# rahul003/dmlc-core

Hardware: AMD Instinct MI355X
Metric: parsed rows/sec (LibSVM->CSR in device memory), aggregate over GPUs (higher is better)
Workload: dtype fp32 values / u32 indices (text parse, no matmul)

## Files before the change

### src/gpu/tile_kernels.hip

```cpp
#include <dmlc/gpu/hip_utils.h>
#include <hip/hip_runtime.h>

#include <cstdlib>
#include <type_traits>

#include "../data/strtonum.h"
#include "./device_common.h"
#include "./kernels.h"
#include "./token_decode.h"

namespace dmlc {
namespace gpu {

namespace {
constexpr int kThreads = 256;
constexpr int kSub = static_cast<int>(kTileBytes / 4096);
constexpr unsigned kOffBits = 13;
constexpr unsigned kMaxTileTokens = static_cast<unsigned>(kTileBytes / 2);
static_assert(kTileBytes == 8192, "entry packing assumes 8 KiB tiles");

__device__ __forceinline__ uint32_t gather_hi(uint32_t z) {
  return __builtin_amdgcn_udot4(z, 0x08040201u, 0u, false) >> 7;
}

// ... 23 lines not shown
  for (int i = 0; i < 4; ++i) m |= gather_hi((w[i] << 1) & 0x80808080u) << (4 * i);
  return m;
}

__device__ __forceinline__ bool num_start(uint32_t c) {
  return (c >= '0' && c <= '9') || c == '+' || c == '-' || c == '.';
}

template <bool kCheck, bool kFull = false, bool kCheckTokens = true>
__device__ __forceinline__ bool lane_masks(uint4 v, uint32_t pc, size_t pos, size_t n,
                                           uint32_t* lm, uint32_t* tm) {
  uint32_t sep, eol, ctl;
  classify16(v, &sep, &eol, &ctl);
  const uint32_t prev_eol = (pc == '\n' || pc == '\r') ? 1u : 0u;
  const uint32_t prev_sep = (prev_eol || pc == ' ' || pc == '\t') ? 1u : 0u;
  uint32_t valid = 0xFFFFu;
  if (kFull) {
  } else if (pos >= n) {
    valid = 0;
  } else if (n - pos < 16) {
    valid = (1u << (n - pos)) - 1u;
  }
  *lm = ~eol & ((eol << 1) | prev_eol) & valid & 0xFFFFu;
  *tm = ~sep & ((sep << 1) | prev_sep) & valid & 0xFFFFu;
  if (!kCheck) return false;
  bool bad = (*lm & ~*tm) != 0;
  uint32_t t = kCheckTokens ? *tm : 0u;
  while (t != 0) {
    const int j = __ffs(t) - 1;
    t &= t - 1;
    bad |= !num_start(dev::vec_byte(v, j));
  }
  uint32_t c = ctl & valid;
  while (c != 0) {
    const int j = __ffs(c) - 1;
    c &= c - 1;
    bad |= !((0x2600u >> dev::vec_byte(v, j)) & 1u);
  }
  return bad;
}

__device__ __forceinline__ uint4 load16(const uint8_t* __restrict__ text, size_t pos, size_t n) {
  if (pos < n) return *reinterpret_cast<const uint4*>(text + pos);
  return make_uint4(0, 0, 0, 0);
}

__device__ __forceinline__ uint32_t prev_byte(const uint8_t* __restrict__ text, size_t pos,
                                              uint4 v) {
  const uint32_t from_left = dev::lane_shr1(v.w >> 24);
  if (dev::lane_id() != 0) return from_left;
  return pos == 0 ? static_cast<uint32_t>('\n') : text[pos - 1];
}

template <bool kFull>
__device__ __forceinline__ bool count16(uint4 v, uint32_t pc, size_t pos, size_t n,
                                        uint32_t* lines, uint32_t* toks, uint32_t* qtoks,
                                        uint32_t* packed = nullptr) {
  const uint32_t w[4] = {v.x, v.y, v.z, v.w};
  uint32_t acc_t[2] = {0u, 0u}, acc_l[2] = {0u, 0u};
  const size_t room = kFull ? 16 : (pos >= n ? 0 : (n - pos < 16 ? n - pos : 16));
  uint32_t prev_sep = (pc <= 0x20u) ? 0x80u : 0u;
  uint32_t prev_eol = (pc == '\n' || pc == '\r') ? 0x80u : 0u;
  bool bad = false;
  uint32_t blank = 0;
#pragma unroll
  for (int i = 0; i < 4; ++i) {
    const uint32_t x = w[i];
    const uint32_t lo7 = x & 0x7F7F7F7Fu;
    const uint32_t le20 = ~((lo7 + 0x5F5F5F5Fu) | x) & 0x80808080u;
    const uint32_t lt20 = ~((lo7 + 0x60606060u) | x) & 0x80808080u;
    const uint32_t b6 = ((x & 0x06060606u) + 0x7E7E7E7Eu) & 0x80808080u;
    const int valid_bytes = static_cast<int>(room) - 4 * i;
    const uint32_t valid = valid_bytes >= 4 ? 0x80808080u
                           : (valid_bytes <= 0 ? 0u : (0x80808080u >> (8 * (4 - valid_bytes))));
    const uint32_t sep = le20 | (~valid & 0x80808080u);
    const uint32_t eol = le20 & b6;
    const uint32_t sep_before = (sep << 8) | prev_sep;
    const uint32_t eol_before = (eol << 8) | prev_eol;
    const uint32_t tm = ~sep & sep_before & 0x80808080u;
    const uint32_t lm = ~eol & eol_before & valid & 0x80808080u;
    *qtoks += __popc(tm & (x << 1));
    const uint32_t wgt = (i & 1) ? 0x80402010u : 0x08040201u;
    acc_t[i >> 1] = __builtin_amdgcn_udot4(tm, wgt, acc_t[i >> 1], false);
    acc_l[i >> 1] = __builtin_amdgcn_udot4(lm, wgt, acc_l[i >> 1], false);
    blank |= lm & ~tm;
    uint32_t c = lt20 & valid;
    while (c != 0) {
      const int j = (__ffs(c) - 1) >> 3;
      c &= c - 1;
      bad |= !((0x2600u >> ((x >> (8 * j)) & 0xFFu)) & 1u);
    }
    prev_sep = (sep >> 24) & 0x80u;
    prev_eol = (eol >> 24) & 0x80u;
  }
  const uint32_t pt = (acc_t[0] >> 7) | (acc_t[1] << 1);
  const uint32_t pl = (acc_l[0] >> 7) | (acc_l[1] << 1);
  *toks += __popc(pt);
  *lines += __popc(pl);
  bad |= blank != 0;
  if (packed != nullptr) *packed = pt | (pl << 16);
  return bad;
}

template <bool kFull>
__device__ __forceinline__ uint32_t lines16(uint4 v, uint32_t pc, int room) {
  const uint32_t w[4] = {v.x, v.y, v.z, v.w};
  uint32_t prev_eol = (pc == '\n' || pc == '\r') ? 0x80u : 0u;
  uint32_t lines = 0;
#pragma unroll
  for (int i = 0; i < 4; ++i) {
    const uint32_t x = w[i];
    const uint32_t lo7 = x & 0x7F7F7F7Fu;
    const uint32_t le20 = ~((lo7 + 0x5F5F5F5Fu) | x) & 0x80808080u;
    const uint32_t b6 = ((x & 0x06060606u) + 0x7E7E7E7Eu) & 0x80808080u;
    const uint32_t eol = le20 & b6;
    const int valid_bytes = room - 4 * i;
    const uint32_t valid = kFull || valid_bytes >= 4
                               ? 0x80808080u
                               : (valid_bytes <= 0 ? 0u : (0x80808080u >> (8 * (4 - valid_bytes))));
    lines += __popc(~eol & ((eol << 8) | prev_eol) & valid);
    prev_eol = (eol >> 24) & 0x80u;
  }
  return lines;
}

__device__ __forceinline__ uint64_t lookback_lines(uint64_t* st, size_t tile, uint32_t own,
                                                   uint32_t tag, int lane) {
  const uint64_t tg = static_cast<uint64_t>(tag) << 34;
  if (lane == 0) {
    __hip_atomic_store(&st[tile], tg | ((tile == 0 ? 2ull : 1ull) << 32) | own, __ATOMIC_RELAXED,
                       __HIP_MEMORY_SCOPE_AGENT);
  }
  if (tile == 0) return 0;
  uint64_t excl = 0;
  int64_t j = static_cast<int64_t>(tile) - 1;
  for (;;) {
    const int64_t k = j - lane;
    const uint64_t v = k >= 0 ? __hip_atomic_load(&st[k], __ATOMIC_RELAXED, __HIP_MEMORY_SCOPE_AGENT)
                              : (tg | (2ull << 32));
    const uint32_t state = static_cast<uint32_t>(v >> 32) & 3u;
    const bool ready = (v >> 34) == tag && state != 0;
    const uint64_t inc = __ballot(ready && state == 2u);
    const uint64_t waiting = __ballot(!ready);
    const int first = inc != 0 ? __builtin_ctzll(inc) : dev::kWave - 1;
    const uint64_t need = first >= dev::kWave - 1 ? ~0ull : ((2ull << first) - 1ull);
    if ((waiting & need) != 0) {
      __builtin_amdgcn_s_sleep(1);
      continue;
    }
    excl += dev::wave_sum(lane <= first ? static_cast<uint32_t>(v) : 0u);
    if (inc != 0) break;
    j -= dev::kWave;
  }
  if (lane == 0) {
    __hip_atomic_store(&st[tile], tg | (2ull << 32) | (excl + own), __ATOMIC_RELAXED,
                       __HIP_MEMORY_SCOPE_AGENT);
  }
  return excl;
}

constexpr int kCountLoads = static_cast<int>(kTileBytes / 1024);
__global__ __launch_bounds__(kThreads) void k_tile_count(const uint8_t* __restrict__ text,
                                                         size_t n, size_t ntiles,
                                                         uint64_t* __restrict__ counts,
                                                         uint32_t* __restrict__ flags,
                                                         uint2* __restrict__ masks) {
  const int lane = dev::lane_id();
  const size_t tile = static_cast<size_t>(blockIdx.x) * (kThreads / dev::kWave) +
                      threadIdx.x / dev::kWave;
  if (tile >= ntiles) return;
  const size_t base = tile * kTileBytes;
  uint4 v[kCountLoads];
#pragma unroll
  for (int j = 0; j < kCountLoads; ++j) v[j] = load16(text, base + j * 1024 + lane * 16, n);
  const uint32_t first = base == 0 ? static_cast<uint32_t>('\n') : text[base - 1];
  uint32_t lines = 0, toks = 0, qtoks = 0;
  bool bad = false;
  uint2* const mrow = masks + tile * (kTileBytes / 2048) * dev::kWave + lane;
  auto count_tile = [&](auto full) {
    uint32_t m0 = 0;
#pragma unroll
    for (int j = 0; j < kCountLoads; ++j) {
      const uint32_t left = dev::lane_shr1(v[j].w >> 24);
      const uint32_t wrap = j == 0 ? first : dev::lane63(v[j - 1].w >> 24);
      const uint32_t pc = lane == 0 ? wrap : left;
      uint32_t m;
      bad |= count16<decltype(full)::value>(v[j], pc, base + j * 1024 + lane * 16, n, &lines,
                                            &toks, &qtoks, &m);
      if (j & 1) {
        mrow[(j >> 1) * dev::kWave] = make_uint2(m0, m);
      } else {
        m0 = m;
      }
    }
  };
  if (base + kTileBytes <= n) {
    count_tile(std::true_type{});
  } else {
    count_tile(std::false_type{});
  }
  lines = dev::wave_sum(lines);
  toks = dev::wave_sum(toks);
  qtoks = dev::wave_sum(qtoks);
  const bool any_bad = __any(bad);
  if (lane == 0) {
    counts[tile] = (static_cast<uint64_t>(lines) << 32) | (toks - qtoks);
    flags[tile] = (any_bad ? kFlagIrregular : 0u) | (qtoks != 0 ? kFlagQid : 0u);
  }
}

__device__ __forceinline__ void publish_host_meta(ChunkMeta* host_meta, ChunkMeta m) {
  m.pad = 0;
  *host_meta = m;
  __threadfence_system();
  *reinterpret_cast<volatile unsigned*>(&host_meta->pad) = 1u;
}

constexpr int kScanThreads = 1024;
constexpr int kScanPer = 8;

__global__ __launch_bounds__(kScanThreads) void k_tile_scan(uint64_t* __restrict__ counts,
                                                            const uint32_t* __restrict__ flags,
                                                            size_t ntiles, ChunkMeta* meta,
                                                            ChunkMeta* host_meta, int raw) {
  __shared__ uint64_t swave[kScanThreads / 64];
  __shared__ uint32_t sflag[kScanThreads / 64];
  const int wid = threadIdx.x / dev::kWave;
  uint64_t carry = 0;
  uint32_t fl = 0;
  for (size_t t0 = 0; t0 < ntiles; t0 += static_cast<size_t>(kScanThreads) * kScanPer) {
    const size_t base = t0 + static_cast<size_t>(threadIdx.x) * kScanPer;
    uint64_t v[kScanPer];
    uint64_t s = 0;
#pragma unroll
    for (int i = 0; i < kScanPer; ++i) {
      v[i] = base + i < ntiles ? counts[base + i] : 0;
      if (base + i < ntiles) fl |= flags[base + i];
      s += v[i];
    }
    uint64_t wtot;
    const uint64_t wx = dev::wave_excl_scan(s, &wtot);
    if (dev::lane_id() == 0) swave[wid] = wtot;
    __syncthreads();
    uint64_t before = 0, all = 0;
#pragma unroll
    for (int w = 0; w < kScanThreads / 64; ++w) {
      const uint64_t t = swave[w];
      if (w < wid) before += t;
      all += t;
    }
    uint64_t x = carry + before + wx;
#pragma unroll
    for (int i = 0; i < kScanPer; ++i) {
      if (base + i < ntiles) counts[base + i] = x;
      x += v[i];
    }
// ... 340 lines not shown
__device__ __forceinline__ void list_slice(uint32_t* sl, uint32_t tm, uint32_t lm, uint32_t at,
                                           uint32_t base, uint32_t line0, int lane) {
  uint32_t m = tm;
#pragma unroll
  for (int t = 0; t < 2; ++t) {
    const uint32_t j = static_cast<uint32_t>(__builtin_ctz(m | 0x10000u));
    const bool has = m != 0;
    sl[has ? at : kCap + lane] = list_entry(j & 15u, lm, base, line0);
    at += has ? 1u : 0u;
    m &= m - 1;
  }
  if (__any(m != 0)) {
    for (; m != 0; m &= m - 1) {
      sl[at++] = list_entry(static_cast<uint32_t>(__builtin_ctz(m)), lm, base, line0);
    }
  }
}

__device__ __forceinline__ uint32_t round_slot(int lane) {
  const uint32_t l = static_cast<uint32_t>(lane) & 31u;
  uint32_t k;
  if (l < 4) {
    k = l;
  } else if (l < 12) {
    k = 16u + (l - 4u);
  } else if (l < 16) {
    k = 4u + (l - 12u);
  } else if (l < 20) {
    k = 24u + (l - 16u);
  } else if (l < 28) {
    k = 8u + (l - 20u);
  } else {
    k = 28u + (l - 28u);
  }
  return (static_cast<uint32_t>(lane) & 32u) + k;
}

struct FillPass {
  uint64_t* status;
  unsigned long long* ticket;
  unsigned long long ticket0;
  ChunkMeta* meta;
  uint32_t exp;
  const uint32_t* masks;
};

template <TextFormat F, typename IndexType, bool kOnePass, bool kLean = false>
__global__ __launch_bounds__(kThreads, DMLC_FILL_WAVES) void k_tile_fill(
    const uint8_t* __restrict__ text, size_t n, size_t ntiles, const uint64_t* __restrict__ prefix,
    FillTarget<IndexType> out, MetaPartial* __restrict__ partials, FillPass op) {
  __shared__ uint4 s_text[kFillWaves][kStageVecs];
  __shared__ uint32_t s_list[kFillWaves][kListCap + 64];
  __shared__ uint32_t s_dq[kFillWaves][kQueueCap];
  const int wave = __builtin_amdgcn_readfirstlane(threadIdx.x / dev::kWave);
  const int lane = dev::lane_id();
  size_t group = blockIdx.x;
  if constexpr (kOnePass) {
    __shared__ uint32_t s_ticket;
    if (threadIdx.x == 0) s_ticket = static_cast<uint32_t>(atomicAdd(op.ticket, 1ull) - op.ticket0);
    __syncthreads();
    group = s_ticket;
  }
  const size_t tile = group * kFillWaves + wave;
  if (tile >= ntiles) return;
  uint4* const st = s_text[wave];
  uint32_t* const sl = s_list[wave];
  uint32_t* const dq = s_dq[wave];
  uint32_t qh = 0, qn = 0;
  const uint32_t slot = round_slot(lane);
  const size_t tile0 = tile * kTileBytes;

  const __amdgpu_buffer_rsrc_t trs = text_rsrc(text + tile0, n - tile0);
  const uint32_t loff = static_cast<uint32_t>(lane) * 16;
  uint4 a = bload16(trs, loff);
  uint4 b = bload16(trs, loff + 1024);
  uint4 t = make_uint4(0, 0, 0, 0);
  if (!kOnePass && lane < 4) t = bload16(trs, loff + kStepBytes);
  __amdgpu_buffer_rsrc_t mrs;
  const uint32_t moff = static_cast<uint32_t>(lane) * 8;
  uint2 mk = make_uint2(0, 0);
  if constexpr (!kOnePass) {
    mrs = mask_rsrc(op.masks, tile, ntiles);
    mk = load_masks(mrs, moff, 0);
  }
  uint32_t carry_pc = 0;
  if constexpr (kOnePass) carry_pc = tile0 == 0 ? static_cast<uint32_t>('\n') : text[tile0 - 1];
  uint64_t line_base, tok_base;
  unsigned count_flags = 0;
  if constexpr (kOnePass) {
    uint4 v[kCountLoads];
    v[0] = a;
    v[1] = b;
#pragma unroll
    for (int j = 2; j < kCountLoads; ++j) v[j] = bload16(trs, loff + j * 1024);
    if (lane < 4) t = v[2];
    uint32_t lines = 0, toks = 0, qtoks = 0;
    bool bad = false;
    auto count_tile = [&](auto full) {
#pragma unroll
      for (int j = 0; j < kCountLoads; ++j) {
        const uint32_t left = dev::lane_shr1(v[j].w >> 24);
        const uint32_t wrap = j == 0 ? carry_pc : dev::lane63(v[j - 1].w >> 24);
        const uint32_t pc = lane == 0 ? wrap : left;
        bad |= count16<decltype(full)::value>(v[j], pc, tile0 + j * 1024 + lane * 16, n, &lines,
                                              &toks, &qtoks);
      }
    };
    if (tile0 + kTileBytes <= n) {
      count_tile(std::true_type{});
    } else {
      count_tile(std::false_type{});
    }
    lines = dev::wave_sum(lines);
    const uint32_t ent = dev::wave_sum(toks - qtoks);
    qtoks = dev::wave_sum(qtoks);
    count_flags = (__any(bad) ? kFlagIrregular : 0u) | (qtoks != 0 ? kFlagQid : 0u);
    const uint64_t own = (static_cast<uint64_t>(lines) << 31) | ent;
    const uint64_t excl = dev::lookback_pairs<31>(op.status, tile, own, lane);
    line_base = excl >> 31;
    tok_base = excl & 0x7FFFFFFFull;
    if (tile + 1 == ntiles && lane == 0) {
      ChunkMeta m;
      m.nlines = m.nrows = line_base + lines;
      m.nnz = tok_base + ent - (line_base + lines);
      m.max_index = m.max_field = 0;
      m.flags = 0;
      m.pad = 0;
      *op.meta = m;
    }
  } else {
    const uint64_t pre = prefix[tile];
    line_base = pre >> 32;
    tok_base = pre & 0xffffffffull;
  }
  const uint64_t C = out.nnz_base + tok_base - line_base;
  const uint64_t R = out.row_base + line_base;
  auto clamp32 = [](int64_t v) {
    return static_cast<int32_t>(v > INT32_MAX ? INT32_MAX : (v < INT32_MIN ? INT32_MIN : v));
  };
  const int32_t nnz_room =
      clamp32(static_cast<int64_t>(out.nnz_limit) - static_cast<int64_t>(C));
  const int32_t row_room =
      clamp32(static_cast<int64_t>(out.row_limit) - static_cast<int64_t>(R));
  const uint32_t nnz_room_u = nnz_room > 0 ? static_cast<uint32_t>(nnz_room) : 0u;
  IndexType* const idx_at = out.index + C;
  float* const val_at = out.value + C;
  IndexType* const fld_at = out.field != nullptr ? out.field + C : nullptr;
  float* const lab_at = out.label + R - 1;
  uint64_t* const off_at = out.offset + R - 1;
  float* const wgt_at = !kLean && out.weight != nullptr ? out.weight + R - 1 : nullptr;
  uint64_t* const qid_at = !kLean && out.qid != nullptr ? out.qid + R - 1 : nullptr;
  const bool qid_chunk = !kLean && F == TextFormat::kLibSVM && out.qid != nullptr;

  uint32_t tok0 = 0;
  uint32_t lcnt = 0;
  uint32_t carry = 0;
  uint32_t qid_prev = 0;
  using MaxT = typename std::conditional<sizeof(IndexType) == 4, uint32_t, uint64_t>::type;
  MaxT mx_index = 0, mx_field = 0;
  bool any_value = false, any_weight = false, irregular = false, neg = false, need_w = false;
  bool over = false;
  uint32_t sink = 0;

#pragma unroll 1
  for (int s = 0; s < kSteps; ++s) {
    const bool last = s + 1 == kSteps;
    const size_t pos_a = tile0 + s * kStepBytes + lane * 16;
    if (tile0 + static_cast<size_t>(s + 1) * kStepBytes + 64 > n) {
// ... 119 lines not shown
      const uint32_t voff = static_cast<uint32_t>(rel) * 4u;
      auto at = [](auto* base, uint32_t off) {
        using T = typename std::remove_pointer<decltype(base)>::type;
        return reinterpret_cast<T*>(reinterpret_cast<char*>(base) + off);
      };
      if constexpr (F == TextFormat::kLibSVM) {
        if (feat) {
          *at(idx_at, boff) = static_cast<IndexType>(u0);
          *at(val_at, voff) = t.r == 2 ? t.f0 : 1.0f;
        }
        any_value |= feat && t.r == 2;
        const MaxT iu = static_cast<MaxT>(static_cast<IndexType>(u0));
        mx_index = feat && iu > mx_index ? iu : mx_index;
      } else {
        const uint64_t u1 = (static_cast<uint64_t>(t.u1_hi) << 32) | t.u1;
        if (feat) {
          *at(fld_at, boff) = static_cast<IndexType>(u0);
          *at(idx_at, boff) = static_cast<IndexType>(u1);
          *at(val_at, voff) = t.r == 3 ? t.f0 : 1.0f;
        }
        any_value |= feat && t.r == 3;
        const MaxT iu = static_cast<MaxT>(static_cast<IndexType>(u1));
        const MaxT fu = static_cast<MaxT>(static_cast<IndexType>(u0));
        mx_index = feat && iu > mx_index ? iu : mx_index;
        mx_field = feat && fu > mx_field ? fu : mx_field;
      }
      neg |= active && bad;
    };
    auto enqueue = [&](bool defer, uint32_t li) {
      const uint64_t dm = __ballot(defer);
      if (dm != 0) {
        const uint32_t rank = static_cast<uint32_t>(__popcll(dm & ((1ull << lane) - 1ull)));
        if (defer) dq[(qh + qn + rank) & (kQueueCap - 1)] = li;
        qn += static_cast<uint32_t>(__popcll(dm));
      }
    };
    for (uint32_t r0 = 0;;) {
      const bool qround = qn >= static_cast<uint32_t>(dev::kWave) || (r0 >= ndec && qn != 0);
      if (!qround && r0 >= ndec) break;
      if (!qround && r0 + 2 * dev::kWave <= ndec) {
        const uint32_t la = r0 + slot, lb = la + dev::kWave;
        const uint32_t ea = sl[la], eb = sl[lb];
        tok::Token ta, tb;
        ta.u0_hi = ta.u1_hi = tb.u0_hi = tb.u1_hi = 0;
        ta.u1 = tb.u1 = 0;
        bool oka, okb;
        if (dev::pricing_exp(op.exp) & 2u) {
          ta.u0 = ea;
          tb.u0 = eb;
          ta.f0 = ta.f1 = tb.f0 = tb.f1 = 1.0f;
          ta.r = tb.r = 2;
          oka = okb = true;
        } else {
          tok::decode2<F>(st, ea & 0x1FFFu, eb & 0x1FFFu, ((ea >> 13) & 1u) != 0,
                          ((eb >> 13) & 1u) != 0, &ta, &tb, &oka, &okb);
        }
        enqueue(!oka, la);
        enqueue(!okb, lb);
        emit(oka, ea, tok0 + la, ta, false);
        emit(okb, eb, tok0 + lb, tb, false);
        r0 += 2 * dev::kWave;
        continue;
      }
      bool active;
      uint32_t e, i;
      tok::Token t;
      t.u0_hi = t.u1_hi = 0;
      t.u1 = 0;
      bool bad = false;
      if (!qround) {
        const uint32_t li = r0 + slot;
        active = li < ndec;
        e = active ? sl[li] : 0u;
        i = tok0 + li;
        const bool is_label = active && ((e >> 13) & 1u) != 0;
        const bool ok = tok::decode<F>(st, e & 0x1FFFu, is_label, &t);
        enqueue(active & !ok, li);
        active = active & ok;
        r0 += dev::kWave;
      } else {
        dev::wave_sync();
        const uint32_t cnt = qn < static_cast<uint32_t>(dev::kWave) ? qn : dev::kWave;
        active = slot < cnt;
        const uint32_t li = active ? dq[(qh + slot) & (kQueueCap - 1)] : 0u;
        qh += cnt;
        qn -= cnt;
        e = active ? sl[li] : 0u;
        i = tok0 + li;
        const bool is_label = active && ((e >> 13) & 1u) != 0;
        const uint32_t off = e & 0x1FFFu;
        bool ok = false;
        if (active) {
          const tok::ExtToken x = tok::decode_ext<F>(
              st, off, is_label, off >= kSlotBytes ? 2 * kSlotBytes : kSlotBytes);
          t = x.t;
          ok = x.ok;
        }
        if (active & !ok) {
          const uint32_t in_slot = off >= kSlotBytes ? 1u : 0u;
          const int step = in_slot == (static_cast<uint32_t>(s) & 1u) ? s : s - 1;
          const size_t gpos =
              tile0 + static_cast<size_t>(step) * kStepBytes + off - in_slot * kSlotBytes;
          const GenericResult g = generic_token<F, IndexType>(text, n, gpos, is_label);
          t = g.t;
          bad = g.bad;
          irregular |= !num_start(text[gpos]);
        }
      }
      emit(active, e, i, t, bad);
    }
    const uint32_t left = total - ndec;
    const uint32_t moved = lane < static_cast<int>(left) ? sl[ndec + lane] : 0u;
    dev::wave_sync();
    if (lane < static_cast<int>(left)) sl[lane] = moved;
    tok0 += ndec;
    carry = left;
    lcnt += nline;
    dev::wave_sync();
  }
  unsigned fl = count_flags;
  if (sink == 0x9E3779B9u) fl |= kFlagIrregular;
  if (any_value) fl |= kFlagValue;
  if (any_weight) fl |= kFlagWeight;
  if (irregular) fl |= kFlagIrregular;
  if (neg) fl |= kFlagNegIndex;
  if (kLean ? any_weight : need_w) fl |= kFlagNeedWeight;
  if (over) fl |= kFlagOverflow;
  if (F == TextFormat::kLibFM) fl |= kFlagField;
  const unsigned long long mi = dev::wave_max(static_cast<unsigned long long>(mx_index));
  const unsigned long long mf = dev::wave_max(static_cast<unsigned long long>(mx_field));
  fl = dev::wave_or(fl);
  if (lane == 0) {
    MetaPartial p;
    p.max_index = mi;
    p.max_field = mf;
    p.flags = fl;
    p.pad = 0;
    partials[tile] = p;
  }
}

struct HashTarget {
  void* x;
  float* label;
  uint64_t row_base;
  uint64_t nlines;
  int dim;
  float scale;
  uint32_t seed;
  uint32_t tag;
  uint64_t* status;
  unsigned long long* ticket;
  unsigned long long ticket0;
  uint64_t row_cap;
  ChunkMeta* meta;
  const uint32_t* masks;
};

__device__ __forceinline__ uint32_t owned_tokens(uint32_t tm, uint32_t lm, uint32_t L0,
                                                 uint32_t own) {
  uint32_t m = tm;
  if (L0 == 0) m &= lm != 0 ? ~((lm & (0u - lm)) - 1u) : 0u;
  const uint32_t nl = static_cast<uint32_t>(__popc(lm));
  if (L0 + nl > own) {
    if (L0 > own) return 0u;
    uint32_t x = lm;
    for (uint32_t k = own - L0; k != 0; --k) x &= x - 1u;
    m &= (x & (0u - x)) - 1u;
  }
  return m;
}

template <TextFormat F, typename IndexType, bool kFP8, bool kOnePass>
__global__ __launch_bounds__(kThreads, DMLC_FILL_WAVES) void k_tile_hash(
    const uint8_t* __restrict__ text, size_t n, size_t ntiles,
    const uint64_t* __restrict__ prefix, HashTarget out, MetaPartial* __restrict__ partials) {
  __shared__ uint4 s_text[kFillWaves][kHashText / 16];
  __shared__ uint32_t s_list[kFillWaves][kHashListCap + 64];
  extern __shared__ __attribute__((aligned(16))) float s_hrow[];
  const int wave = __builtin_amdgcn_readfirstlane(threadIdx.x / dev::kWave);
  const int lane = dev::lane_id();
  size_t group = blockIdx.x;
  if constexpr (kOnePass) {
    __shared__ uint32_t s_ticket;
    if (threadIdx.x == 0) s_ticket = static_cast<uint32_t>(atomicAdd(out.ticket, 1ull) - out.ticket0);
    __syncthreads();
    group = s_ticket;
  }
  const size_t tile = group * kFillWaves + wave;
  if (tile >= ntiles) return;
  uint4* const st = s_text[wave];
  uint32_t* const sl = s_list[wave];
  const int dim = out.dim;
  float* const row = s_hrow + static_cast<size_t>(wave) * dim;
  const uint32_t slot = round_slot(lane);
  const size_t tile0 = tile * kTileBytes;
  const __amdgpu_buffer_rsrc_t trs = text_rsrc(text + tile0, n - tile0);
  const uint32_t loff = static_cast<uint32_t>(lane) * 16;
  uint4 a = bload16(trs, loff);
  uint4 b = bload16(trs, loff + 1024);
  __amdgpu_buffer_rsrc_t mrs;
  const uint32_t moff = static_cast<uint32_t>(lane) * 8;
  uint2 mk = make_uint2(0, 0);
  if constexpr (!kOnePass) {
    mrs = mask_rsrc(out.masks, tile, ntiles);
    mk = load_masks(mrs, moff, 0);
  }
  uint32_t carry_pc = 0;
  if constexpr (kOnePass) carry_pc = tile0 == 0 ? static_cast<uint32_t>('\n') : text[tile0 - 1];
  uint64_t line_base;
  uint32_t own;
  if constexpr (kOnePass) {
    uint4 v[kCountLoads];
    v[0] = a;
    v[1] = b;
#pragma unroll
    for (int j = 2; j < kCountLoads; ++j) v[j] = bload16(trs, loff + j * 1024);
    const bool full = tile0 + kTileBytes <= n;
    uint32_t lines = 0;
#pragma unroll
    for (int j = 0; j < kCountLoads; ++j) {
      const uint32_t left = dev::lane_shr1(v[j].w >> 24);
      const uint32_t wrap = j == 0 ? carry_pc : dev::lane63(v[j - 1].w >> 24);
      const uint32_t pc = lane == 0 ? wrap : left;
      if (full) {
        lines += lines16<true>(v[j], pc, 16);
      } else {
        const size_t pos = tile0 + j * 1024 + lane * 16;
        const int room = pos >= n ? 0 : (n - pos < 16 ? static_cast<int>(n - pos) : 16);
        lines += lines16<false>(v[j], pc, room);
      }
    }
    own = dev::wave_sum(lines);
    line_base = lookback_lines(out.status, tile, own, out.tag, lane);
    if (tile + 1 == ntiles && lane == 0) {
      ChunkMeta m;
      m.nlines = m.nrows = line_base + own;
      m.nnz = 0;
      m.max_index = m.max_field = 0;
      m.flags = 0;
      m.pad = 0;
      *out.meta = m;
    }
  } else {
    line_base = prefix[tile] >> 32;
// ... 128 lines not shown
        const uint32_t b32 = dev::wave_excl_scan<uint32_t>(static_cast<uint32_t>(cnt), &t32);
        before = (before & ~0xFFFFFFFFull) | b32;
        tot = (tot & ~0xFFFFFFFFull) | t32;
      }
      const uint32_t ntok_a = static_cast<uint32_t>(tot & 0xFFFFu);
      const uint32_t ntok = ntok_a + static_cast<uint32_t>((tot >> 16) & 0xFFFFu);
      const uint32_t ntok_b = ntok - ntok_a;
      const bool split = carry + ntok > kHashListCap;
      if (split && (carry + ntok_a > kHashListCap || ntok_b > kHashListCap)) {
        irregular = true;
        break;
      }
      lcnt += nline;
      const bool eol_end = carry_pc == '\n' || carry_pc == '\r';
      const bool last = nxt >= n || lcnt > own || (s + 1 >= kSteps && lcnt == own && eol_end);
      if (!last) {
        const uint32_t so = static_cast<uint32_t>(s + 1) * kStepBytes;
        a = bload16(trs, loff + so);
        b = bload16(trs, loff + so + 1024);
        if (lane < 4) t = bload16(trs, loff + so + kStepBytes);
        if constexpr (!kOnePass) mk = load_masks(mrs, moff, s + 1);
      }

      list_slice<kHashListCap>(sl, tm_a, lm_a, carry + static_cast<uint32_t>(before & 0xFFFFu),
                               sbase + lane * 16, la0, lane);
      const uint32_t pk_m = tm_b | (lm_b << 16);
      const uint32_t pk_o = static_cast<uint32_t>((before >> 16) & 0xFFFFu) | (lb0 << 16);
      if (!split) {
        list_slice<kHashListCap>(sl, tm_b, lm_b,
                                 carry + ntok_a + static_cast<uint32_t>((before >> 16) & 0xFFFFu),
                                 sbase + 1024 + lane * 16, lb0, lane);
      }
      dev::wave_sync();
      uint32_t total = 0, ndec = 0;
#pragma unroll 1
      for (int part = 0;; ++part) {
        total = !split ? carry + ntok : (part == 0 ? carry + ntok_a : ntok_b);
        uint32_t rest = (last || (split && part == 0)) ? 0u : total % dev::kWave;
        if (rest != 0 && (dev::uniform(sl[total - rest]) & 0x1FFFu) < kHashText - kHashCarry - 64u) {
          rest = 0;
        }
        ndec = total - rest;
        for (uint32_t r0 = 0; r0 < ndec; r0 += dev::kWave) {
          const uint32_t li = r0 + slot;
          const bool active = li < ndec;
          const uint32_t e = active ? sl[li] : 0u;
          const bool is_label = active && ((e >> 13) & 1u) != 0;
          const uint32_t off = e & 0x1FFFu;
          const uint32_t lc = e >> 14;
          tok::Token t;
          t.u0_hi = t.u1_hi = 0;
          t.u1 = 0;
          bool bad = false;
          bool ok = tok::decode<F>(st, off, is_label, &t);
          if (__any(active & !ok)) {
            if (active & !ok) {
              const tok::ExtToken x = tok::decode_ext<F>(st, off, is_label, kHashText);
              if (x.ok) t = x.t;
              ok = x.ok;
            }
          }
          if (active & !ok) {
            const size_t gpos = cur + off - sbase;
            const GenericResult gr = generic_token<F, IndexType>(text, n, gpos, is_label);
            t = gr.t;
            bad = gr.bad;
            irregular |= !num_start(text[gpos]);
          }
          if (active & is_label && (!kOnePass || R + lc - 1 < row_cap)) lab_at[lc] = t.f0;
          bool feat = active & !is_label;
          uint64_t key;
          float val;
          const uint64_t u0 = (static_cast<uint64_t>(t.u0_hi) << 32) | t.u0;
          if constexpr (F == TextFormat::kLibSVM) {
            key = static_cast<uint64_t>(static_cast<IndexType>(u0));
            val = t.r == 2 ? t.f0 : 1.0f;
          } else {
            const uint64_t u1 = (static_cast<uint64_t>(t.u1_hi) << 32) | t.u1;
            feat &= t.r >= 2;
            key = dev::hash_key(static_cast<uint64_t>(static_cast<IndexType>(u1)),
                                static_cast<uint64_t>(static_cast<IndexType>(u0)), true);
            val = t.r == 3 ? t.f0 : 1.0f;
          }
          neg |= active && bad;
          const uint32_t h = dev::hash_u64(key, out.seed);
          uint32_t bucket;
          if (pow2) {
            bucket = h & dmask;
          } else {
            bucket = h % static_cast<uint32_t>(dim);
          }
          const float sv = (h & 0x80000000u) ? -val : val;
          const uint32_t lo = dev::uniform(sl[r0] >> 14);
          const uint32_t hi =
              dev::uniform(sl[r0 + dev::kWave - 1 < ndec ? r0 + dev::kWave - 1 : ndec - 1] >> 14);
          for (uint32_t rr = lo; rr <= hi; ++rr) {
            if (rr != open) {
              if (open != 0) flush(open);
              open = rr;
            }
            if (feat && lc == rr) atomicAdd(&row[bucket], sv);
          }
        }
        if (!split || part == 1) break;
        carry = 0;
        dev::wave_sync();
        list_slice<kHashListCap>(sl, pk_m & 0xFFFFu, pk_m >> 16, pk_o & 0xFFFFu,
// ... 283 lines not shown
```

### src/gpu/token_decode.h

```cpp
#ifndef DMLC_SRC_GPU_TOKEN_DECODE_H_
#define DMLC_SRC_GPU_TOKEN_DECODE_H_

#include <hip/hip_runtime.h>

#include <cstdint>

#include "./kernels.h"

namespace dmlc {
namespace gpu {
namespace tok {

__device__ __forceinline__ uint4 ext16(const uint4* lds, uint32_t a) {
  const uint32_t* w = reinterpret_cast<const uint32_t*>(lds) + (a >> 2);
  const uint32_t w0 = w[0], w1 = w[1], w2 = w[2], w3 = w[3], w4 = w[4];
  const uint32_t r = a & 3u;
  return make_uint4(__builtin_amdgcn_alignbyte(w1, w0, r), __builtin_amdgcn_alignbyte(w2, w1, r),
                    __builtin_amdgcn_alignbyte(w3, w2, r), __builtin_amdgcn_alignbyte(w4, w3, r));
}

__device__ __forceinline__ uint32_t pow10_u(uint32_t k) {
  const uint32_t a = (k & 1u) ? 10u : 1u;
  const uint32_t b = (k & 2u) ? 100u : 1u;
  const uint32_t c = (k & 4u) ? 10000u : 1u;
  return __umul24(__umul24(a, b), c);
}

__device__ __forceinline__ void pow10f(uint32_t k, float* p, float* inv) {
  *p = static_cast<float>(pow10_u(k));
  const bool b0 = (k & 1u) != 0, b1 = (k & 2u) != 0, b2 = (k & 4u) != 0;
  float a0 = b0 ? 0.1f : 1.0f, a1 = b0 ? 0.001f : 0.01f;
  float a2 = b0 ? 1e-5f : 1e-4f, a3 = b0 ? 1e-7f : 1e-6f;
  asm("" : "+v"(a0), "+v"(a1), "+v"(a2), "+v"(a3));
  float c0 = b1 ? a1 : a0, c1 = b1 ? a3 : a2;
  asm("" : "+v"(c0), "+v"(c1));
  *inv = b2 ? c1 : c0;
}

__device__ __forceinline__ uint3 ext12(const uint4* lds, uint32_t a) {
  const uint32_t* w = reinterpret_cast<const uint32_t*>(lds) + (a >> 2);
  const uint32_t w0 = w[0], w1 = w[1], w2 = w[2], w3 = w[3];
  const uint32_t r = a & 3u;
  return make_uint3(__builtin_amdgcn_alignbyte(w1, w0, r), __builtin_amdgcn_alignbyte(w2, w1, r),
                    __builtin_amdgcn_alignbyte(w3, w2, r));
}

struct Run8 {
  uint32_t k, val, term;
};

__device__ __forceinline__ Run8 digit_run8(uint32_t lo, uint32_t hi, uint32_t next) {
  const uint32_t t0 = lo ^ 0x30303030u, t1 = hi ^ 0x30303030u;
  const uint32_t b0 = (((t0 & 0x7F7F7F7Fu) + 0x76767676u) | t0) & 0x80808080u;
  const uint32_t b1 = (((t1 & 0x7F7F7F7Fu) + 0x76767676u) | t1) & 0x80808080u;
  const uint64_t bad = (static_cast<uint64_t>(b1) << 32) | b0;
  const uint32_t c8 = static_cast<uint32_t>(__builtin_ctzg(bad, 64)) & ~7u;
  const uint32_t half = 32u - (c8 >> 1);
  const uint64_t t = (static_cast<uint64_t>(t1) << 32) | t0;
  const uint64_t x = (t << half) << half;
  const uint32_t xl = static_cast<uint32_t>(x), xh = static_cast<uint32_t>(x >> 32);
  const uint32_t p0 = __builtin_amdgcn_udot4(xl, 0x0000010Au, 0u, false);
  const uint32_t p1 = __builtin_amdgcn_udot4(xl, 0x010A0000u, 0u, false);
  const uint32_t p2 = __builtin_amdgcn_udot4(xh, 0x0000010Au, 0u, false);
  const uint32_t p3 = __builtin_amdgcn_udot4(xh, 0x010A0000u, 0u, false);
  const uint32_t v = __umul24(__umul24(__umul24(p0, 100u) + p1, 100u) + p2, 100u) + p3;
  Run8 r;
  r.k = c8 >> 3;
  r.val = v;
  const uint64_t raw = (static_cast<uint64_t>(hi) << 32) | lo;
  r.term = c8 < 64 ? static_cast<uint32_t>(raw >> c8) & 0xFFu : next;
  return r;
}

__device__ __forceinline__ bool is_end(uint32_t c) {
  return c <= 32u && ((0x100002601ull >> c) & 1u) != 0;
}

struct Num {
  uint32_t ival;
  float fval;
  uint32_t end, term;
  bool ok_float, ok_uint;
};

__device__ __forceinline__ Num parse_num(const uint4* lds, uint32_t a) {
#if defined(__clang__)
#pragma clang fp contract(off)
#endif
  Num o;
  const uint3 g = ext12(lds, a);
  const uint32_t c0 = g.x & 0xFFu;
  const bool neg = c0 == '-';
  const uint32_t s = (neg || c0 == '+') ? 1u : 0u;
  const uint32_t h0 = __builtin_amdgcn_alignbyte(g.y, g.x, s);
  const uint32_t h1 = __builtin_amdgcn_alignbyte(g.z, g.y, s);
  const uint32_t nb = (__builtin_amdgcn_alignbyte(g.z, g.y, s + 1u) >> 24);
  const Run8 ir = digit_run8(h0, h1, nb);
  const uint32_t k = ir.k;
  const bool dot = ir.term == '.';
  const uint32_t fa = a + s + k + 1u;
  const uint3 f = ext12(lds, fa);
  const Run8 fr = digit_run8(f.x, f.y, f.z & 0xFFu);
  uint32_t nf = fr.k;
  o.ok_float = (k <= 7) & (dot ? ((nf <= 7) & ((k | nf) != 0)) : k != 0);
  o.ok_uint = (s == 0) & !dot & (k != 0) & !((k == 8) & (ir.term - '0' < 10u));
  o.term = dot ? fr.term : ir.term;
  o.end = dot ? fa + nf : a + s + k;
  o.ival = ir.val;
  float p, inv;
  pow10f(nf, &p, &inv);
  const float ff = static_cast<float>(fr.val);
  const float q0 = ff * inv;
  const float rem = __builtin_fmaf(-q0, p, ff);
  float frac = __builtin_fmaf(rem, inv, q0);
  const bool longf = dot & (nf == 8u);
  if (__any(longf)) {
    const uint3 f2 = ext12(lds, fa + 8u);
    const Run8 r2 = digit_run8(f2.x, f2.y, f2.z & 0xFFu);
    if (longf) {
      nf = 8u + r2.k;
      const uint64_t fv = static_cast<uint64_t>(fr.val) * pow10_u(r2.k) + r2.val;
      frac = static_cast<float>(static_cast<double>(fv) /
                                (1e8 * static_cast<double>(pow10_u(r2.k))));
      o.ok_float = (k <= 7) & (nf < 16u);
      o.term = r2.term;
      o.end = fa + nf;
    }
  }
  float v = static_cast<float>(ir.val);
  v = dot ? v + frac : v;
  const bool has_e = (o.term == 'e') | (o.term == 'E');
  if (__any(has_e & o.ok_float)) {
    const uint3 e = ext12(lds, o.end + 1u);
    const uint32_t cs = e.x & 0xFFu;
    const bool eneg = cs == '-';
    const uint32_t es = (cs == '-' || cs == '+') ? 1u : 0u;
    const Run8 er = digit_run8(__builtin_amdgcn_alignbyte(e.y, e.x, es),
                               __builtin_amdgcn_alignbyte(e.z, e.y, es), 0u);
    const uint32_t ex = er.val;
    if (has_e) {
      const float scale = ex <= 7u ? static_cast<float>(pow10_u(ex))
                                   : (ex == 8u ? 1e8f : (ex == 9u ? 1e9f : 1e10f));
      o.ok_float = o.ok_float & (er.k < 4u) & (ex <= 10u);
      o.end = o.end + 1u + es + er.k;
      o.term = er.term;
      v = eneg ? (v / scale) : (v * scale);
    }
  }
  o.fval = neg ? -v : v;
  return o;
}

__device__ __forceinline__ Num parse_int(const uint4* lds, uint32_t a) {
  Num o;
  const uint3 g = ext12(lds, a);
  const uint32_t c0 = g.x & 0xFFu;
  const bool neg = c0 == '-';
  const uint32_t s = (neg || c0 == '+') ? 1u : 0u;
  const uint32_t h0 = __builtin_amdgcn_alignbyte(g.y, g.x, s);
  const uint32_t h1 = __builtin_amdgcn_alignbyte(g.z, g.y, s);
  const uint32_t nb = (__builtin_amdgcn_alignbyte(g.z, g.y, s + 1u) >> 24);
  const Run8 ir = digit_run8(h0, h1, nb);
  const uint32_t k = ir.k;
  const bool dot = ir.term == '.';
  o.ok_float = (k <= 7) & (k != 0) & !dot;
  o.ok_uint = (s == 0) & !dot & (k != 0) & !((k == 8) & (ir.term - '0' < 10u));
  o.term = ir.term;
  o.end = a + s + k;
  o.ival = ir.val;
  const float v = static_cast<float>(ir.val);
  o.fval = neg ? -v : v;
  return o;
}


struct Token {
  uint32_t u0, u1;
  uint32_t u0_hi, u1_hi;
  float f0, f1;
  int r;
};

template <TextFormat F>
__device__ __forceinline__ bool assemble(const Num& n1, const Num& n2, const Num& n3,
                                         bool is_label, Token* t) {
  const bool c1 = n1.term == ':';
  const bool first = is_label ? n1.ok_float : n1.ok_uint;
  const bool pair_ok = first & (c1 ? (n2.ok_float & is_end(n2.term)) : is_end(n1.term));
  t->u0 = n1.ival;
  t->f1 = n2.fval;
  if (F == TextFormat::kLibSVM) {
    t->f0 = is_label ? n1.fval : n2.fval;
    t->r = c1 ? 2 : 1;
    return pair_ok;
  }
  const bool c2 = n2.term == ':';
  const bool triple_ok =
      c1 & n1.ok_uint & n2.ok_uint & (c2 ? (n3.ok_float & is_end(n3.term)) : is_end(n2.term));
  t->u1 = n2.ival;
  t->f0 = is_label ? n1.fval : n3.fval;
  t->r = is_label ? (c1 ? 2 : 1) : (c2 ? 3 : 2);
  return is_label ? pair_ok : triple_ok;
}

template <TextFormat F>
__device__ __forceinline__ bool decode(const uint4* lds, uint32_t a, bool is_label, Token* t) {
  Num n1 = parse_int(lds, a);
  if (__any(is_label & (n1.term == '.'))) n1 = parse_num(lds, a);
  const bool c1 = n1.term == ':';
  Num n2, n3;
  if (F == TextFormat::kLibSVM) {
    n2 = parse_num(lds, n1.end + (c1 ? 1u : 0u));
    n3 = n2;
  } else {
    n2 = parse_int(lds, n1.end + (c1 ? 1u : 0u));
    if (__any(is_label & c1 & (n2.term == '.'))) n2 = parse_num(lds, n1.end + (c1 ? 1u : 0u));
    const bool c2 = n2.term == ':';
    n3 = parse_num(lds, n2.end + (c2 ? 1u : 0u));
  }
  return assemble<F>(n1, n2, n3, is_label, t);
}

template <TextFormat F>
__device__ __forceinline__ void decode2(const uint4* lds, uint32_t a0, uint32_t a1, bool lab0,
                                        bool lab1, Token* t0, Token* t1, bool* ok0, bool* ok1) {
  Num n1a = parse_int(lds, a0);
  Num n1b = parse_int(lds, a1);
  if (__any((lab0 & (n1a.term == '.')) | (lab1 & (n1b.term == '.')))) {
    n1a = parse_num(lds, a0);
    n1b = parse_num(lds, a1);
  }
  const uint32_t s2a = n1a.end + (n1a.term == ':' ? 1u : 0u);
  const uint32_t s2b = n1b.end + (n1b.term == ':' ? 1u : 0u);
  Num n2a, n2b, n3a, n3b;
  if (F == TextFormat::kLibSVM) {
    n2a = parse_num(lds, s2a);
    n2b = parse_num(lds, s2b);
    n3a = n2a;
    n3b = n2b;
  } else {
    n2a = parse_int(lds, s2a);
    n2b = parse_int(lds, s2b);
    if (__any((lab0 & (n1a.term == ':') & (n2a.term == '.')) |
              (lab1 & (n1b.term == ':') & (n2b.term == '.')))) {
      n2a = parse_num(lds, s2a);
      n2b = parse_num(lds, s2b);
    }
    n3a = parse_num(lds, n2a.end + (n2a.term == ':' ? 1u : 0u));
    n3b = parse_num(lds, n2b.end + (n2b.term == ':' ? 1u : 0u));
  }
  *ok0 = assemble<F>(n1a, n2a, n3a, lab0, t0);
  *ok1 = assemble<F>(n1b, n2b, n3b, lab1, t1);
}

__device__ __forceinline__ uint32_t win_dw(uint4 g0, uint4 g1, uint32_t q) {
  return q < 4 ? (q < 2 ? (q == 0 ? g0.x : g0.y) : (q == 2 ? g0.z : g0.w))
               : (q < 6 ? (q == 4 ? g1.x : g1.y) : (q == 6 ? g1.z : g1.w));
}

__device__ __forceinline__ uint32_t win_byte(uint4 g0, uint4 g1, uint32_t i) {
  return (win_dw(g0, g1, i >> 2) >> (8u * (i & 3u))) & 0xFFu;
}

__device__ __forceinline__ uint32_t win_word(uint4 g0, uint4 g1, uint32_t i) {
  const uint32_t q = i >> 2;
  return __builtin_amdgcn_alignbyte(win_dw(g0, g1, q < 7 ? q + 1 : 7u), win_dw(g0, g1, q), i & 3u);
}

struct ExtNum {
  float fval;
  uint32_t end, term;
  bool ok;
};

__device__ __forceinline__ ExtNum parse_num_ext(const uint4* lds, uint32_t a, uint32_t limit) {
#if defined(__clang__)
#pragma clang fp contract(off)
#endif
  ExtNum o;
  const uint3 g = ext12(lds, a);
  const uint32_t c0 = g.x & 0xFFu;
  const bool neg = c0 == '-';
  const uint32_t s = (neg || c0 == '+') ? 1u : 0u;
  const uint32_t h0 = __builtin_amdgcn_alignbyte(g.y, g.x, s);
  const uint32_t h1 = __builtin_amdgcn_alignbyte(g.z, g.y, s);
  const uint32_t nb = __builtin_amdgcn_alignbyte(g.z, g.y, s + 1u) >> 24;
  const Run8 ir = digit_run8(h0, h1, nb);
  const uint32_t k = ir.k;
  const bool dot = ir.term == '.';
  const uint32_t fa = a + s + k + 1u;
  const uint3 f1 = ext12(lds, fa);
  const Run8 r1 = digit_run8(f1.x, f1.y, f1.z & 0xFFu);
  const uint3 f2 = ext12(lds, fa + 8u);
  const Run8 r2 = digit_run8(f2.x, f2.y, f2.z & 0xFFu);
  const bool two = r1.k == 8u;
  const uint32_t nf = dot ? (two ? 8u + r2.k : r1.k) : 0u;
  const uint32_t after = dot ? fa + nf : a + s + k;
  const uint32_t cterm = dot ? (two ? r2.term : r1.term) : ir.term;
  const bool has_e = cterm == 'e' || cterm == 'E';
  const uint3 e = ext12(lds, after + 1u);
  const uint32_t cs = e.x & 0xFFu;
  const bool eneg = cs == '-';
// ... 109 lines not shown
```

Baseline: 175.8 million.

## Defer control-byte validation to cold path and use LDS pow10 table in decode

The count pass no longer runs a per-byte loop for control characters. It accumulates a cheap SWAR mask of suspicious control bytes and re-scans the tile with the exact check only when some lane flags one. Token boundary masks now use alignbit instead of shift/or/mask, and the blank-line check works on the packed masks. The fill and hash kernels fill a small per-wave LDS table of powers of ten, replacing computed pow10f in parse_num, and is_end/assemble are simplified. This costs extra LDS per wave and a re-read of the tile from global memory when control bytes appear.

```diff
diff --git a/src/gpu/tile_kernels.hip b/src/gpu/tile_kernels.hip
--- a/src/gpu/tile_kernels.hip
+++ b/src/gpu/tile_kernels.hip
@@ -99,54 +99,83 @@
   return pos == 0 ? static_cast<uint32_t>('\n') : text[pos - 1];
 }
 
+struct CountAcc {
+  uint32_t lines = 0, toks = 0, qtoks = 0;
+  uint32_t blank = 0;
+  uint32_t ctl = 0;
+};
+
 template <bool kFull>
-__device__ __forceinline__ bool count16(uint4 v, uint32_t pc, size_t pos, size_t n,
-                                        uint32_t* lines, uint32_t* toks, uint32_t* qtoks,
+__device__ __forceinline__ void count16(uint4 v, uint32_t pc, size_t pos, size_t n, CountAcc* acc,
                                         uint32_t* packed = nullptr) {
   const uint32_t w[4] = {v.x, v.y, v.z, v.w};
   uint32_t acc_t[2] = {0u, 0u}, acc_l[2] = {0u, 0u};
   const size_t room = kFull ? 16 : (pos >= n ? 0 : (n - pos < 16 ? n - pos : 16));
-  uint32_t prev_sep = (pc <= 0x20u) ? 0x80u : 0u;
-  uint32_t prev_eol = (pc == '\n' || pc == '\r') ? 0x80u : 0u;
-  bool bad = false;
-  uint32_t blank = 0;
+  uint32_t sep_prev = (pc <= 0x20u) ? 0x80000000u : 0u;
+  uint32_t eol_prev = (pc == '\n' || pc == '\r') ? 0x80000000u : 0u;
 #pragma unroll
   for (int i = 0; i < 4; ++i) {
     const uint32_t x = w[i];
     const uint32_t lo7 = x & 0x7F7F7F7Fu;
     const uint32_t le20 = ~((lo7 + 0x5F5F5F5Fu) | x) & 0x80808080u;
-    const uint32_t lt20 = ~((lo7 + 0x60606060u) | x) & 0x80808080u;
-    const uint32_t b6 = ((x & 0x06060606u) + 0x7E7E7E7Eu) & 0x80808080u;
+    const uint32_t b6 = (x & 0x06060606u) + 0x7E7E7E7Eu;
     const int valid_bytes = static_cast<int>(room) - 4 * i;
     const uint32_t valid = valid_bytes >= 4 ? 0x80808080u
                            : (valid_bytes <= 0 ? 0u : (0x80808080u >> (8 * (4 - valid_bytes))));
-    const uint32_t sep = le20 | (~valid & 0x80808080u);
+    const uint32_t sep = kFull ? le20 : le20 | (~valid & 0x80808080u);
     const uint32_t eol = le20 & b6;
-    const uint32_t sep_before = (sep << 8) | prev_sep;
-    const uint32_t eol_before = (eol << 8) | prev_eol;
-    const uint32_t tm = ~sep & sep_before & 0x80808080u;
-    const uint32_t lm = ~eol & eol_before & valid & 0x80808080u;
-    *qtoks += __popc(tm & (x << 1));
+    const uint32_t sep_before = __builtin_amdgcn_alignbit(sep, sep_prev, 24);
+    const uint32_t eol_before = __builtin_amdgcn_alignbit(eol, eol_prev, 24);
+    const uint32_t tm = ~sep & sep_before;
+    const uint32_t lm = kFull ? ~eol & eol_before : ~eol & eol_before & valid;
+    acc->qtoks += __popc(tm & (x << 1));
     const uint32_t wgt = (i & 1) ? 0x80402010u : 0x08040201u;
     acc_t[i >> 1] = __builtin_amdgcn_udot4(tm, wgt, acc_t[i >> 1], false);
     acc_l[i >> 1] = __builtin_amdgcn_udot4(lm, wgt, acc_l[i >> 1], false);
-    blank |= lm & ~tm;
-    uint32_t c = lt20 & valid;
-    while (c != 0) {
-      const int j = (__ffs(c) - 1) >> 3;
-      c &= c - 1;
-      bad |= !((0x2600u >> ((x >> (8 * j)) & 0xFFu)) & 1u);
-    }
-    prev_sep = (sep >> 24) & 0x80u;
-    prev_eol = (eol >> 24) & 0x80u;
+    const uint32_t u = lo7 ^ 0x0A0A0A0Au;
+    const uint32_t ctl = (u + 0x7F7F7F7Fu) & ~(u + 0x60606060u) & ~x;
+    acc->ctl |= kFull ? ctl : ctl & valid;
+    sep_prev = sep;
+    eol_prev = eol;
   }
   const uint32_t pt = (acc_t[0] >> 7) | (acc_t[1] << 1);
   const uint32_t pl = (acc_l[0] >> 7) | (acc_l[1] << 1);
-  *toks += __popc(pt);
-  *lines += __popc(pl);
-  bad |= blank != 0;
+  acc->toks += __popc(pt);
+  acc->lines += __popc(pl);
+  acc->blank |= pl & ~pt;
   if (packed != nullptr) *packed = pt | (pl << 16);
+}
+
+__device__ __forceinline__ bool tile_ctl_bad(const uint8_t* __restrict__ text, size_t base,
+                                             size_t n, int lane) {
+  bool bad = false;
+#pragma unroll 1
+  for (int j = 0; j < static_cast<int>(kTileBytes / 1024); ++j) {
+    const size_t pos = base + j * 1024 + lane * 16;
+    const uint4 v = load16(text, pos, n);
+    const int room = pos >= n ? 0 : (n - pos < 16 ? static_cast<int>(n - pos) : 16);
+    const uint32_t w[4] = {v.x, v.y, v.z, v.w};
+#pragma unroll
+    for (int i = 0; i < 4; ++i) {
+      const uint32_t x = w[i];
+      const uint32_t lt20 = ~(((x & 0x7F7F7F7Fu) + 0x60606060u) | x) & 0x80808080u;
+      const int valid_bytes = room - 4 * i;
+      const uint32_t valid = valid_bytes >= 4 ? 0x80808080u
+                             : (valid_bytes <= 0 ? 0u : (0x80808080u >> (8 * (4 - valid_bytes))));
+      uint32_t c = lt20 & valid;
+      while (c != 0) {
+        const int k = (__ffs(c) - 1) >> 3;
+        c &= c - 1;
+        bad |= !((0x2600u >> ((x >> (8 * k)) & 0xFFu)) & 1u);
+      }
+    }
+  }
   return bad;
+}
+
+__device__ __noinline__ bool tile_ctl_bad_cold(const uint8_t* __restrict__ text, size_t base,
+                                               size_t n, int lane) {
+  return tile_ctl_bad(text, base, n, lane);
 }
 
 template <bool kFull>
@@ -221,8 +250,7 @@
 #pragma unroll
   for (int j = 0; j < kCountLoads; ++j) v[j] = load16(text, base + j * 1024 + lane * 16, n);
   const uint32_t first = base == 0 ? static_cast<uint32_t>('\n') : text[base - 1];
-  uint32_t lines = 0, toks = 0, qtoks = 0;
-  bool bad = false;
+  CountAcc acc;
   uint2* const mrow = masks + tile * (kTileBytes / 2048) * dev::kWave + lane;
   auto count_tile = [&](auto full) {
     uint32_t m0 = 0;
@@ -232,8 +260,7 @@
       const uint32_t wrap = j == 0 ? first : dev::lane63(v[j - 1].w >> 24);
       const uint32_t pc = lane == 0 ? wrap : left;
       uint32_t m;
-      bad |= count16<decltype(full)::value>(v[j], pc, base + j * 1024 + lane * 16, n, &lines,
-                                            &toks, &qtoks, &m);
+      count16<decltype(full)::value>(v[j], pc, base + j * 1024 + lane * 16, n, &acc, &m);
       if (j & 1) {
         mrow[(j >> 1) * dev::kWave] = make_uint2(m0, m);
       } else {
@@ -246,9 +273,11 @@
   } else {
     count_tile(std::false_type{});
   }
-  lines = dev::wave_sum(lines);
-  toks = dev::wave_sum(toks);
-  qtoks = dev::wave_sum(qtoks);
+  const uint32_t lines = dev::wave_sum(acc.lines);
+  const uint32_t toks = dev::wave_sum(acc.toks);
+  const uint32_t qtoks = dev::wave_sum(acc.qtoks);
+  bool bad = acc.blank != 0;
+  if (__any((acc.ctl & 0x80808080u) != 0)) bad |= tile_ctl_bad(text, base, n, lane);
   const bool any_bad = __any(bad);
   if (lane == 0) {
     counts[tile] = (static_cast<uint64_t>(lines) << 32) | (toks - qtoks);
@@ -695,6 +724,7 @@
   __shared__ uint4 s_text[kFillWaves][kStageVecs];
   __shared__ uint32_t s_list[kFillWaves][kListCap + 64];
   __shared__ uint32_t s_dq[kFillWaves][kQueueCap];
+  __shared__ float2 s_p10[kFillWaves][tok::kPow10Entries];
   const int wave = __builtin_amdgcn_readfirstlane(threadIdx.x / dev::kWave);
   const int lane = dev::lane_id();
   size_t group = blockIdx.x;
@@ -709,6 +739,8 @@
   uint4* const st = s_text[wave];
   uint32_t* const sl = s_list[wave];
   uint32_t* const dq = s_dq[wave];
+  float2* const p10 = s_p10[wave];
+  tok::pow10_fill(p10, lane);
   uint32_t qh = 0, qn = 0;
   const uint32_t slot = round_slot(lane);
   const size_t tile0 = tile * kTileBytes;
@@ -737,16 +769,14 @@
 #pragma unroll
     for (int j = 2; j < kCountLoads; ++j) v[j] = bload16(trs, loff + j * 1024);
     if (lane < 4) t = v[2];
-    uint32_t lines = 0, toks = 0, qtoks = 0;
-    bool bad = false;
+    CountAcc acc;
     auto count_tile = [&](auto full) {
 #pragma unroll
       for (int j = 0; j < kCountLoads; ++j) {
         const uint32_t left = dev::lane_shr1(v[j].w >> 24);
         const uint32_t wrap = j == 0 ? carry_pc : dev::lane63(v[j - 1].w >> 24);
         const uint32_t pc = lane == 0 ? wrap : left;
-        bad |= count16<decltype(full)::value>(v[j], pc, tile0 + j * 1024 + lane * 16, n, &lines,
-                                              &toks, &qtoks);
+        count16<decltype(full)::value>(v[j], pc, tile0 + j * 1024 + lane * 16, n, &acc);
       }
     };
     if (tile0 + kTileBytes <= n) {
@@ -754,9 +784,11 @@
     } else {
       count_tile(std::false_type{});
     }
-    lines = dev::wave_sum(lines);
-    const uint32_t ent = dev::wave_sum(toks - qtoks);
-    qtoks = dev::wave_sum(qtoks);
+    bool bad = acc.blank != 0;
+    if (__any((acc.ctl & 0x80808080u) != 0)) bad |= tile_ctl_bad_cold(text, tile0, n, lane);
+    const uint32_t lines = dev::wave_sum(acc.lines);
+    const uint32_t ent = dev::wave_sum(acc.toks - acc.qtoks);
+    const uint32_t qtoks = dev::wave_sum(acc.qtoks);
     count_flags = (__any(bad) ? kFlagIrregular : 0u) | (qtoks != 0 ? kFlagQid : 0u);
     const uint64_t own = (static_cast<uint64_t>(lines) << 31) | ent;
     const uint64_t excl = dev::lookback_pairs<31>(op.status, tile, own, lane);
@@ -982,8 +1014,8 @@
           ta.r = tb.r = 2;
           oka = okb = true;
         } else {
-          tok::decode2<F>(st, ea & 0x1FFFu, eb & 0x1FFFu, ((ea >> 13) & 1u) != 0,
-                          ((eb >> 13) & 1u) != 0, &ta, &tb, &oka, &okb);
+          tok::decode2<F, true>(st, ea & 0x1FFFu, eb & 0x1FFFu, ((ea >> 13) & 1u) != 0,
+                                ((eb >> 13) & 1u) != 0, &ta, &tb, &oka, &okb, p10);
         }
         enqueue(!oka, la);
         enqueue(!okb, lb);
@@ -1004,7 +1036,7 @@
         e = active ? sl[li] : 0u;
         i = tok0 + li;
         const bool is_label = active && ((e >> 13) & 1u) != 0;
-        const bool ok = tok::decode<F>(st, e & 0x1FFFu, is_label, &t);
+        const bool ok = tok::decode<F, true>(st, e & 0x1FFFu, is_label, &t, p10);
         enqueue(active & !ok, li);
         active = active & ok;
         r0 += dev::kWave;
@@ -1107,6 +1139,7 @@
     const uint64_t* __restrict__ prefix, HashTarget out, MetaPartial* __restrict__ partials) {
   __shared__ uint4 s_text[kFillWaves][kHashText / 16];
   __shared__ uint32_t s_list[kFillWaves][kHashListCap + 64];
+  __shared__ float2 s_p10[kFillWaves][tok::kPow10Entries];
   extern __shared__ __attribute__((aligned(16))) float s_hrow[];
   const int wave = __builtin_amdgcn_readfirstlane(threadIdx.x / dev::kWave);
   const int lane = dev::lane_id();
@@ -1121,6 +1154,8 @@
   if (tile >= ntiles) return;
   uint4* const st = s_text[wave];
   uint32_t* const sl = s_list[wave];
+  float2* const p10 = s_p10[wave];
+  tok::pow10_fill(p10, lane);
   const int dim = out.dim;
   float* const row = s_hrow + static_cast<size_t>(wave) * dim;
   const uint32_t slot = round_slot(lane);
@@ -1355,7 +1390,7 @@
           t.u0_hi = t.u1_hi = 0;
           t.u1 = 0;
           bool bad = false;
-          bool ok = tok::decode<F>(st, off, is_label, &t);
+          bool ok = tok::decode<F, true>(st, off, is_label, &t, p10);
           if (__any(active & !ok)) {
             if (active & !ok) {
               const tok::ExtToken x = tok::decode_ext<F>(st, off, is_label, kHashText);
diff --git a/src/gpu/token_decode.h b/src/gpu/token_decode.h
--- a/src/gpu/token_decode.h
+++ b/src/gpu/token_decode.h
@@ -35,6 +35,14 @@
   float c0 = b1 ? a1 : a0, c1 = b1 ? a3 : a2;
   asm("" : "+v"(c0), "+v"(c1));
   *inv = b2 ? c1 : c0;
+}
+
+constexpr int kPow10Entries = 9;
+
+__device__ __forceinline__ void pow10_fill(float2* tbl, int lane) {
+  float p, inv;
+  pow10f(static_cast<uint32_t>(lane), &p, &inv);
+  if (lane < kPow10Entries) tbl[lane] = make_float2(p, inv);
 }
 
 __device__ __forceinline__ uint3 ext12(const uint4* lds, uint32_t a) {
@@ -73,7 +81,7 @@
 }
 
 __device__ __forceinline__ bool is_end(uint32_t c) {
-  return c <= 32u && ((0x100002601ull >> c) & 1u) != 0;
+  return (c <= 32u) & (((0x2601u >> (c & 31u)) & 1u) != 0);
 }
 
 struct Num {
@@ -83,7 +91,9 @@
   bool ok_float, ok_uint;
 };
 
-__device__ __forceinline__ Num parse_num(const uint4* lds, uint32_t a) {
+template <bool kLut = false>
+__device__ __forceinline__ Num parse_num(const uint4* lds, uint32_t a,
+                                         const float2* p10 = nullptr) {
 #if defined(__clang__)
 #pragma clang fp contract(off)
 #endif
@@ -108,7 +118,13 @@
   o.end = dot ? fa + nf : a + s + k;
   o.ival = ir.val;
   float p, inv;
-  pow10f(nf, &p, &inv);
+  if constexpr (kLut) {
+    const float2 pi = p10[nf];
+    p = pi.x;
+    inv = pi.y;
+  } else {
+    pow10f(nf, &p, &inv);
+  }
   const float ff = static_cast<float>(fr.val);
   const float q0 = ff * inv;
   const float rem = __builtin_fmaf(-q0, p, ff);
@@ -186,56 +202,61 @@
                                          bool is_label, Token* t) {
   const bool c1 = n1.term == ':';
   const bool first = is_label ? n1.ok_float : n1.ok_uint;
-  const bool pair_ok = first & (c1 ? (n2.ok_float & is_end(n2.term)) : is_end(n1.term));
+  const bool pair_ok = first & (n2.ok_float | !c1);
+  const uint32_t pair_term = c1 ? n2.term : n1.term;
   t->u0 = n1.ival;
   t->f1 = n2.fval;
   if (F == TextFormat::kLibSVM) {
     t->f0 = is_label ? n1.fval : n2.fval;
     t->r = c1 ? 2 : 1;
-    return pair_ok;
+    return pair_ok & is_end(pair_term);
   }
   const bool c2 = n2.term == ':';
-  const bool triple_ok =
-      c1 & n1.ok_uint & n2.ok_uint & (c2 ? (n3.ok_float & is_end(n3.term)) : is_end(n2.term));
+  const bool triple_ok = c1 & n1.ok_uint & n2.ok_uint & (n3.ok_float | !c2);
+  const uint32_t triple_term = c2 ? n3.term : n2.term;
   t->u1 = n2.ival;
   t->f0 = is_label ? n1.fval : n3.fval;
   t->r = is_label ? (c1 ? 2 : 1) : (c2 ? 3 : 2);
-  return is_label ? pair_ok : triple_ok;
-}
-
-template <TextFormat F>
-__device__ __forceinline__ bool decode(const uint4* lds, uint32_t a, bool is_label, Token* t) {
+  return (is_label ? pair_ok : triple_ok) & is_end(is_label ? pair_term : triple_term);
+}
+
+template <TextFormat F, bool kLut = false>
+__device__ __forceinline__ bool decode(const uint4* lds, uint32_t a, bool is_label, Token* t,
+                                       const float2* p10 = nullptr) {
   Num n1 = parse_int(lds, a);
-  if (__any(is_label & (n1.term == '.'))) n1 = parse_num(lds, a);
+  if (__any(is_label & (n1.term == '.'))) n1 = parse_num<kLut>(lds, a, p10);
   const bool c1 = n1.term == ':';
   Num n2, n3;
   if (F == TextFormat::kLibSVM) {
-    n2 = parse_num(lds, n1.end + (c1 ? 1u : 0u));
+    n2 = parse_num<kLut>(lds, n1.end + (c1 ? 1u : 0u), p10);
     n3 = n2;
   } else {
     n2 = parse_int(lds, n1.end + (c1 ? 1u : 0u));
-    if (__any(is_label & c1 & (n2.term == '.'))) n2 = parse_num(lds, n1.end + (c1 ? 1u : 0u));
+    if (__any(is_label & c1 & (n2.term == '.'))) {
+      n2 = parse_num<kLut>(lds, n1.end + (c1 ? 1u : 0u), p10);
+    }
     const bool c2 = n2.term == ':';
-    n3 = parse_num(lds, n2.end + (c2 ? 1u : 0u));
+    n3 = parse_num<kLut>(lds, n2.end + (c2 ? 1u : 0u), p10);
   }
   return assemble<F>(n1, n2, n3, is_label, t);
 }
 
-template <TextFormat F>
+template <TextFormat F, bool kLut = false>
 __device__ __forceinline__ void decode2(const uint4* lds, uint32_t a0, uint32_t a1, bool lab0,
-                                        bool lab1, Token* t0, Token* t1, bool* ok0, bool* ok1) {
+                                        bool lab1, Token* t0, Token* t1, bool* ok0, bool* ok1,
+                                        const float2* p10 = nullptr) {
   Num n1a = parse_int(lds, a0);
   Num n1b = parse_int(lds, a1);
   if (__any((lab0 & (n1a.term == '.')) | (lab1 & (n1b.term == '.')))) {
-    n1a = parse_num(lds, a0);
-    n1b = parse_num(lds, a1);
+    n1a = parse_num<kLut>(lds, a0, p10);
+    n1b = parse_num<kLut>(lds, a1, p10);
   }
   const uint32_t s2a = n1a.end + (n1a.term == ':' ? 1u : 0u);
   const uint32_t s2b = n1b.end + (n1b.term == ':' ? 1u : 0u);
   Num n2a, n2b, n3a, n3b;
   if (F == TextFormat::kLibSVM) {
-    n2a = parse_num(lds, s2a);
-    n2b = parse_num(lds, s2b);
+    n2a = parse_num<kLut>(lds, s2a, p10);
+    n2b = parse_num<kLut>(lds, s2b, p10);
     n3a = n2a;
     n3b = n2b;
   } else {
@@ -243,11 +264,11 @@
     n2b = parse_int(lds, s2b);
     if (__any((lab0 & (n1a.term == ':') & (n2a.term == '.')) |
               (lab1 & (n1b.term == ':') & (n2b.term == '.')))) {
-      n2a = parse_num(lds, s2a);
-      n2b = parse_num(lds, s2b);
-    }
-    n3a = parse_num(lds, n2a.end + (n2a.term == ':' ? 1u : 0u));
-    n3b = parse_num(lds, n2b.end + (n2b.term == ':' ? 1u : 0u));
+      n2a = parse_num<kLut>(lds, s2a, p10);
+      n2b = parse_num<kLut>(lds, s2b, p10);
+    }
+    n3a = parse_num<kLut>(lds, n2a.end + (n2a.term == ':' ? 1u : 0u), p10);
+    n3b = parse_num<kLut>(lds, n2b.end + (n2b.term == ':' ? 1u : 0u), p10);
   }
   *ok0 = assemble<F>(n1a, n2a, n3a, lab0, t0);
   *ok1 = assemble<F>(n1b, n2b, n3b, lab1, t1);
```

Measured after the change: 177.1 million, median of 3. Within noise of the previous version (+0.7%).
